# AllenNeuralDynamics/aind-smartspim-destripe

Hardware: AMD Instinct MI355X
Metric: 2048x2048 uint16 slices/s destriped (higher is better)
Workload: dtype f32

## Files before the change

### aind_smartspim_destripe_amd/csrc/dsx.hip

```cpp
#include <hip/hip_runtime.h>
#include <dlfcn.h>
#include <math.h>
#include <rccl/rccl.h>
#include <stdio.h>
#include <stdlib.h>
#include <string.h>

#include <string>
#include <vector>

#include "../../include/dsx.h"
#include "dsx_kernels.h"
#include "dsx_retile.h"
#include "dsx_rot90.h"
#include "dsx_pyramid.h"
#include "dsx_stackrank.h"
#include "dsx_volhist.h"
#include "dsx_project.h"
#include "dsx_wavelet.h"
#include "dsx_plan.h"
#include "dsx_chain.h"
#include "dsx_io.h"
#include "dsx_streaks.h"
#include "dsx_lightsheet.h"
// ... 402 lines not shown
  hipLaunchKernelGGL(dsx::k_hist, dim3(blocks, c.nb), dim3(64 * dsx::kHistWaves), 0, hs, a);
  DSX_HIP(hipGetLastError());
  return DSX_OK;
}

template <typename A>
void fill_fwd(A& a, const Chain& c, int l) {
  const dsx_ctx* ctx = c.ctx;
  const dsx::Plan& p = ctx->plan;
  const dsx::LevelPlan& lp = p.lv[l];
  memset(&a, 0, sizeof(a));
  a.in = c.d_in;
  a.in_plane_stride = (long long)p.H * p.W;
  a.ws = c.v.ws;
  a.ws_plane_stride = p.plane_floats;
  a.in_off = (l > 0) ? p.lv[l - 1].aa_off : 0;
  a.H = lp.hin; a.W = lp.win; a.ldin = lp.ldin;
  a.aa_off = lp.aa_off; a.da_off = lp.da_off;
  a.h = lp.h; a.w = lp.w; a.ld = lp.ld; a.lda = lp.lda;
  a.minmax = c.v.minmax;
  a.lvl = l; a.L = p.L;
  a.stats = c.v.stats;
  a.fg_cutoff = ctx->fg_cutoff;
  a.shared = ctx->stack_mode ? 1 : 0;
}

int stage_forward(const Chain& c) {
  dsx_ctx* ctx = c.ctx;
  const dsx::Plan& p = ctx->plan;
  const CohortView& v = c.v;
  const dsx::ChainShape& sh = c.sh;
  hipStream_t s = v.stream;
  const int nb = c.nb;
  for (int l = 0; l < p.L; ++l) {
    if (sh.fuse12 && l == 1) continue;
    if (l >= skips(ctx->tune).from) continue;
    const dsx::LevelPlan& lp = p.lv[l];
    LaunchScope ls(ctx, l == 0 ? KC_FWD1 : KC_FWD);
    if (sh.generic) {
      dsx::GenFwdArgs g;
      fill_fwd(g, c, l);
      g.F = ctx->wl_len;
      memcpy(g.lo, ctx->wl[0], sizeof(float) * ctx->wl_len);
      memcpy(g.hi, ctx->wl[1], sizeof(float) * ctx->wl_len);
      const dim3 gg((lp.w + dsx::kGenTW - 1) / dsx::kGenTW, (lp.h + dsx::kGenTH - 1) / dsx::kGenTH, nb);
      auto kern = level_kernel(l == 0, c.in_dtype, dsx::k_fwd_gen<2>, dsx::k_fwd_gen<0>, dsx::k_fwd_gen<1>);
      hipLaunchKernelGGL(kern, gg, dim3(256), dsx::gen_fwd_lds_bytes(g.F), s, g);
      DSX_HIP(hipGetLastError());
      continue;
    }
    dsx::Fwd1Args f;
    fill_fwd(f, c, l);
    f.ablate = ctx->ablate;
    f.fg_cutoff_u16 = (unsigned)std::min(65536.0, std::max(0.0, ceil((double)ctx->fg_cutoff)));
    const bool fused = sh.fuse12 && l == 0;
    if (fused) {
      const dsx::LevelPlan& l2 = p.lv[1];
      f.aa2_off = l2.aa_off; f.da2_off = l2.da_off;
      f.h2 = l2.h; f.w2 = l2.w; f.ld2 = l2.ld; f.lda2 = l2.lda;
    }
    const dsx::MarchLaunch m = dsx::fwd_launch(p, sh, ctx->tune, ctx->cus, nb, v.alone, l);
    f.nstrips = m.nstrips; f.nseg = m.nseg; f.rows_per_seg = m.rows_per_seg;
    auto kern = (fused && m.wpb == 8) ? pixel_kernel(c.in_dtype, dsx::k_fwd_march<0, true, 8>, dsx::k_fwd_march<1, true, 8>)
                : fused ? pixel_kernel(c.in_dtype, dsx::k_fwd_march<0, true>, dsx::k_fwd_march<1, true>)
                : level_kernel(l == 0, c.in_dtype, dsx::k_fwd_march<2>, dsx::k_fwd_march<0>, dsx::k_fwd_march<1>);
    hipLaunchKernelGGL(kern, dim3(m.grid_x, nb), dim3(64 * m.wpb), 0, s, f);
    DSX_HIP(hipGetLastError());
    if (sh.split && l == 0) {
      DSX_HIP(hipEventRecord(v.ev[0], s));
      DSX_HIP(hipStreamWaitEvent(v.helper, v.ev[0], 0));
      if (int rc = hist_levels(c, 0, 2, v.helper)) return rc;
      DSX_HIP(hipEventRecord(v.ev[1], v.helper));
    }
  }
  return DSX_OK;
}

int stage_thresholds(const Chain& c, int32_t* d_cfg_used) {
  dsx_ctx* ctx = c.ctx;
  const dsx::Plan& p = ctx->plan;
  const CohortView& v = c.v;
  hipStream_t s = v.stream;
  const int L = p.L;
  if (int rc = hist_levels(c, c.sh.split ? 2 : 0, L, s)) return rc;
  if (c.sh.split) DSX_HIP(hipStreamWaitEvent(s, v.ev[1], 0));
  if (L > 0 && c.sh.thresholds) {
    dsx::OtsuArgs a;
    a.stats = v.stats;
    a.npix = (double)p.H * (double)p.W;
    a.high_int = ctx->high_int;
    a.minmax = v.minmax;
    a.hist = v.hist;
    a.thr = v.thr;
    a.otsu = v.otsu;
    a.cfg = v.cfg;
    a.means = v.means;
    a.max_thr[0] = (float)ctx->cfg[0].max_threshold;
    a.max_thr[1] = (float)ctx->cfg[1].max_threshold;
    a.L = L;
    a.sticky = ctx->d_sticky;
    a.shared = ctx->stack_mode ? 1 : 0;
    LaunchScope ls(ctx, KC_OTSU);
    hipLaunchKernelGGL(dsx::k_otsu, dim3(L, c.nb), dim3(64), 0, s, a);
    DSX_HIP(hipGetLastError());
    if (d_cfg_used)
      DSX_HIP(hipMemcpyAsync(d_cfg_used, v.cfg, sizeof(int32_t) * c.nb, hipMemcpyDeviceToDevice, s));
  } else if (d_cfg_used) {
// ... 2477 lines not shown
```

### aind_smartspim_destripe_amd/csrc/dsx_chain.h

```cpp
#ifndef DSX_CHAIN_H
#define DSX_CHAIN_H

#include <stddef.h>
#include <stdlib.h>

#include <algorithm>

#include "dsx_plan.h"

namespace dsx {

constexpr int kMarchCols = 256;
constexpr int kMarchOut = (kMarchCols - 4) / 2;
constexpr int kFuseOut = (kMarchOut - 4) / 2;
constexpr int kHistWaves = 8;
constexpr int kRowMaxWaves = 8;
constexpr int kRowMultiMax = 8;
constexpr int kRowPackMax = 4;
constexpr int kRowPackValues = 18;
constexpr int kWideThreads = 512;
constexpr int kWideCpl = 36;
constexpr int kWideMaxLen = kWideThreads * kWideCpl;
constexpr int kRfWaves = 8;
constexpr int kRfRows = 2 * kRfWaves - 2;
constexpr int kGenTH = 16, kGenTW = 32;
constexpr int kGenOH = 32, kGenOW = 64;
constexpr size_t kLdsLimit = 160 * 1024;
constexpr size_t kC32Bytes = 8;

#ifdef __HIPCC__
#define DSX_CHAIN_HD __host__ __device__
#else
#define DSX_CHAIN_HD
#endif
inline DSX_CHAIN_HD int gen_fwd_cols(int F) { return 2 * kGenTW + F - 2 + 1; }
inline DSX_CHAIN_HD int gen_fwd_rows(int F) { return 2 * kGenTH + F - 2; }
inline size_t gen_fwd_lds_bytes(int F) {
  return sizeof(float) * (size_t)(gen_fwd_rows(F) + 2 * kGenTH) * gen_fwd_cols(F);
}
inline DSX_CHAIN_HD int gen_inv_krows(int F) { return kGenOH / 2 + F / 2 - 1; }
inline DSX_CHAIN_HD int gen_inv_kcols(int F) { return kGenOW / 2 + F / 2 - 1; }
inline size_t gen_inv_lds_bytes(int F) {
  return sizeof(float) * 2 * (size_t)gen_inv_krows(F) * (gen_inv_kcols(F) + 1 + kGenOW + 1);
}

}

struct DsxTuning {
  int row_wpb = 0;
  int march_waves = 256 * 16;
  bool no_quant = false;
  int seg_min_rows = 4;
  bool no_fuse = false;
  bool no_fuse_inv = false;
  bool no_pair = false;
  bool no_fuse_rf = false;
  bool fuse_rf_wide = false;
  int hist_rows = 0;
  int fwd_wpb = 8, inv_wpb = 8;
  bool no_row_multi = false;
  int row_multi_alone = 48;
  bool no_row_pack = false;
  int row_pack = 0;
  int row_pack_wpb = 4;
  int row_pack_fill = 16;
  int helper = -1;
  bool no_pipeline = false;
#ifdef DSX_DIAG
  int skip_hist = 0, skip_row = 0, skip_from = 1000;
#endif
};

namespace dsx {

inline int env_int(const char* name, int fallback) {
  const char* v = getenv(name);
  return (v && *v) ? atoi(v) : fallback;
}

inline void read_tuning(DsxTuning& t) {
  t.row_wpb = env_int("DSX_ROW_WPB", 0);
  if (t.row_wpb != 0) t.row_wpb = std::max(4, std::min(t.row_wpb, (int)kRowMaxWaves));
  t.march_waves = std::max(64, env_int("DSX_MARCH_WAVES", 256 * 16));
  t.no_quant = env_int("DSX_NO_QUANT", 0) != 0;
  t.seg_min_rows = std::max(2, env_int("DSX_SEG_MIN_ROWS", 4));
  t.no_fuse = env_int("DSX_NO_FUSE", 0) != 0;
  t.no_fuse_inv = env_int("DSX_NO_FUSE_INV", 0) != 0;
  t.no_pair = env_int("DSX_NO_PAIR", 0) != 0;
  t.no_fuse_rf = env_int("DSX_NO_FUSE_RF", 0) != 0;
  t.fuse_rf_wide = env_int("DSX_FUSE_RF_WIDE", 0) != 0;
  t.hist_rows = std::max(0, env_int("DSX_HIST_ROWS", 0));
  t.fwd_wpb = env_int("DSX_FWD_WPB", 8) == 4 ? 4 : 8;
  t.inv_wpb = env_int("DSX_INV_WPB", 8) == 4 ? 4 : 8;
  t.no_row_multi = env_int("DSX_NO_ROW_MULTI", 0) != 0;
  t.row_multi_alone = std::max(0, env_int("DSX_ROW_MULTI_ALONE", 48));
  t.no_row_pack = env_int("DSX_NO_ROW_PACK", 0) != 0;
  t.row_pack = std::max(0, std::min(env_int("DSX_ROW_PACK", 0), (int)kRowPackMax));
  t.row_pack_wpb = env_int("DSX_ROW_PACK_WPB", 4) == 8 ? 8 : 4;
  t.row_pack_fill = std::max(0, env_int("DSX_ROW_PACK_FILL", 16));
  t.helper = getenv("DSX_HELPER") ? (env_int("DSX_HELPER", 0) != 0 ? 1 : 0) : -1;
  t.no_pipeline = env_int("DSX_NO_PIPELINE", 0) != 0;
#ifdef DSX_DIAG
  t.skip_hist = env_int("DSX_SKIP_HIST", 0);
  t.skip_row = env_int("DSX_SKIP_ROW", 0);
  t.skip_from = env_int("DSX_SKIP_COARSE", 1000);
#endif
}

struct RowClass {
  bool wide;
  int cpl;
  int gf, nt, halo;
  int plan;
};

struct RowPlan {
  int M, radix[3];
  int cpl;
  int gf, nt, halo;
  bool swz;
};
constexpr int kRowPlanCount = 6;
constexpr RowPlan kRowPlans[kRowPlanCount] = {
    {1026, {19, 9, 6}, 18, 4, 1, 0, false},
    {1071, {17, 9, 7}, 18, 2, 1, 1, false},
    {2048, {16, 16, 8}, 36, 3, 4, 1, true},
    {1815, {15, 11, 11}, 36, 3, 3, 1, false},
    {1024, {16, 8, 8}, 18, 1, 4, 1, true},
    {960, {15, 8, 8}, 18, 1, 4, 1, false},
};
constexpr const RowPlan& row_plan(int id) { return kRowPlans[id - 1]; }

inline RowClass classify_row(int M, int w, int K, int npass, const int* radix) {
  RowClass c = {false, 0, -1, -1, -1, 0};
  const int cpl = (M + 63) / 64;
  if (cpl > 36) { c.wide = true; return c; }
  c.cpl = cpl_class(M);
  const int gf = w >> 8, nt = (w - (gf << 8) + 63) >> 6, halo = K > 0 ? 1 : 0;
  auto set = [&](int plan) { c.gf = gf; c.nt = nt; c.halo = halo; c.plan = plan; };
  for (int id = 1; id <= kRowPlanCount; ++id) {
    const RowPlan& p = row_plan(id);
    if (M == p.M && npass == 3 && radix[0] == p.radix[0] && radix[1] == p.radix[1] && radix[2] == p.radix[2] &&
        c.cpl == p.cpl && gf == p.gf && nt == p.nt && halo == p.halo) {
      set(id);
      return c;
    }
  }
  if (c.cpl == 18 && ((gf == 4 && nt == 1 && halo == 0) || (gf == 2 && nt == 1 && halo == 1))) set(0);
  return c;
}
inline RowClass classify_row(const LevelPlan& lp) { return classify_row(lp.M, lp.w, lp.K, lp.npass, lp.radix); }

inline int rowfinal_plan(const Plan& p, bool in_u16, bool out_u16, bool pair_io, bool wide) {
  const LevelPlan& lp = p.lv[0];
// ... 253 lines not shown
```

### aind_smartspim_destripe_amd/csrc/dsx_kernels.h

```cpp
#ifndef DSX_KERNELS_H
#define DSX_KERNELS_H

#include <type_traits>
#include <hip/hip_runtime.h>
#include <stdint.h>

#include "dsx_chain.h"
#include "dsx_fft_core.h"

#ifdef DSX_DIAG
#define DSX_ABL(a, bits) (((a).ablate & (bits)) != 0)
#else
#define DSX_ABL(a, bits) false
#endif

namespace dsx {

constexpr int kMaxLevels = 16;
constexpr int kMaxPasses = 16;
constexpr int kWave = 64;

#define DSX_DEC_LO                                                                              \
  {0.03522629188570953f, -0.08544127388202666f, -0.13501102001025458f, 0.45987750211849154f,   \
   0.8068915093110925f,  0.33267055295008263f}
// ... 105 lines not shown
}
__device__ __forceinline__ unsigned bit_select(int m, unsigned a, unsigned b) {
  unsigned r;
  asm("v_bfi_b32 %0, %1, %2, %3" : "=v"(r) : "v"(m), "v"(a), "v"(b));
  return r;
}
__device__ __forceinline__ int odd_lane_mask(int lane) {
  int m = -(lane & 1);
  asm("" : "+v"(m));
  return m;
}
__device__ __forceinline__ float bit_select(int m, float a, float b) {
  return as_f32(bit_select(m, as_u32(a), as_u32(b)));
}

__device__ __forceinline__ void wave_sync() {
  __builtin_amdgcn_fence(__ATOMIC_RELEASE, "wavefront");
  __builtin_amdgcn_wave_barrier();
  __builtin_amdgcn_fence(__ATOMIC_ACQUIRE, "wavefront");
}

__device__ __forceinline__ float lane_above(float v) {
  return __builtin_bit_cast(float, __builtin_amdgcn_update_dpp(0, __builtin_bit_cast(int, v), 0x130, 0xF, 0xF, true));
}

__global__ __launch_bounds__(256) void k_zero3(uint4* p0, int n0, uint4* p1, int n1, uint4* p2, int n2) {
  const uint4 z = make_uint4(0u, 0u, 0u, 0u);
  for (int i = blockIdx.x * 256 + threadIdx.x; i < n0 + n1 + n2; i += gridDim.x * 256) {
    if (i < n0) p0[i] = z;
    else if (i < n0 + n1) p1[i - n0] = z;
    else p2[i - n0 - n1] = z;
  }
}

struct Fwd1Args {
  const void* in;
  long long in_plane_stride;
  float* ws;
  long long ws_plane_stride;
  long long in_off;
  int H, W, ldin;
  long long aa_off, da_off;
  int h, w, ld, lda;
  unsigned* minmax;
  int lvl, L;
  PlaneStats* stats;
  float fg_cutoff;
  unsigned fg_cutoff_u16;
  int nstrips, nseg, rows_per_seg;
  long long aa2_off, da2_off;
  int h2, w2, ld2, lda2;
  int ablate;
  int shared;
};

constexpr int kRingRows = 8;
constexpr int kRingPitch = 128;

template <int IN_KIND>
struct MarchStats {
  unsigned cnt = 0;
  unsigned isum_all = 0, isum_fg = 0;
  double fsum_all = 0.0, fsum_fg = 0.0;
  unsigned bad = 0;
  __device__ __forceinline__ void add(float f, float cutoff) {
    if (IN_KIND != 0) bad |= (f > -1.0f && f <= 3.402823466e38f) ? 0u : 1u;
    if (IN_KIND == 0) {
      const unsigned u = (unsigned)f;
      isum_all += u;
      if (f >= cutoff) { isum_fg += u; cnt++; }
    } else {
      fsum_all += (double)f;
      if (f >= cutoff) { fsum_fg += (double)f; cnt++; }
    }
  }
};

struct MarchRaw {
  float4 f;
};

struct MarchCol {
  int gc0;
  int base;
  bool vec;
  bool rev;
  bool dead;
  bool own;
  unsigned own_mask[2];
  int rc[4];
};

__device__ __forceinline__ MarchCol march_col(int gc0, int W, int ld, int w_out, bool lane_owns, bool ext) {
  MarchCol c;
  c.gc0 = gc0;
  c.own = lane_owns;
  c.dead = gc0 > 2 * w_out - 1;
  c.rev = false;
  c.base = gc0;
  const bool aligned = (ld & 3) == 0;
  c.vec = aligned && gc0 >= 0 && gc0 + 3 < W;
  if (ext && aligned && gc0 >= -4 && gc0 + 3 < W + 8) c.vec = true;
  if (!c.vec && !ext && aligned && (W & 3) == 0) {
    if (gc0 + 3 < 0 && -gc0 - 1 < W) { c.base = -gc0 - 4; c.rev = true; c.vec = true; }
    else if (gc0 >= W && 2 * W - 4 - gc0 >= 0) { c.base = 2 * W - 4 - gc0; c.rev = true; c.vec = true; }
  }
// ... 23 lines not shown
      r.f = make_float4(__uint_as_float(u.x), __uint_as_float(u.y), 0.f, 0.f);
    } else {
      const dsx_u32x4 u = __builtin_amdgcn_raw_buffer_load_b128(rs, voff, soff, 0);
      r.f = make_float4(__uint_as_float(u.x), __uint_as_float(u.y), __uint_as_float(u.z), __uint_as_float(u.w));
    }
    return r;
  }
};

template <int IN_KIND, bool FAST>
__device__ __forceinline__ MarchRaw march_issue(const MarchSrc<IN_KIND>& ms, int ld, int H, int gr_raw,
                                                const MarchCol& c) {
  MarchRaw r;
  if (FAST)
    return ms.load((unsigned)(reflect_idx(gr_raw, H) * ld) * MarchSrc<IN_KIND>::ES);
  const void* src = ms.src;
  const long long row = (long long)reflect_idx(gr_raw, H) * ld;
  r.f = make_float4(0.f, 0.f, 0.f, 0.f);
  if (c.dead) return r;
  if (IN_KIND == 0) {
    const uint16_t* p = (const uint16_t*)src + row;
    if (c.vec) {
      const uint2 u = *(const uint2*)(p + c.base);
      r.f.x = __uint_as_float(u.x);
      r.f.y = __uint_as_float(u.y);
    } else {
      const unsigned u0 = p[c.rc[0]], u1 = p[c.rc[1]], u2 = p[c.rc[2]], u3 = p[c.rc[3]];
      r.f.x = __uint_as_float(u0 | (u1 << 16));
      r.f.y = __uint_as_float(u2 | (u3 << 16));
    }
  } else {
    const float* p = (const float*)src + row;
    if (c.vec) r.f = *(const float4*)(p + c.base);
    else r.f = make_float4(p[c.rc[0]], p[c.rc[1]], p[c.rc[2]], p[c.rc[3]]);
  }
  return r;
}

template <int IN_KIND>
__device__ __forceinline__ void march_issue6(const MarchSrc<IN_KIND>& ms, int ld, int H, int g0, const MarchCol& c,
                                             MarchRaw (&out)[6]) {
  constexpr int ES = MarchSrc<IN_KIND>::ES;
  if (g0 >= 0 && g0 + 5 < H) {
    const unsigned pitch = (unsigned)ld * ES;
    unsigned soff = (unsigned)g0 * pitch;
#pragma unroll
    for (int r = 0; r < 6; ++r, soff += pitch) out[r] = ms.load(soff);
  } else {
#pragma unroll
    for (int r = 0; r < 6; ++r) out[r] = march_issue<IN_KIND, true>(ms, ld, H, g0 + r, c);
  }
}

template <int IN_KIND, bool INSIDE = false>
__device__ __forceinline__ void march_consume(const Fwd1Args& a, const MarchRaw& r, int gr_raw, const MarchCol& c,
                                              bool row_in_seg, bool any_rev, MarchStats<IN_KIND>& st,
                                              float (&x)[4]) {
  if (IN_KIND == 0) {
    unsigned u0 = __float_as_uint(r.f.x), u1 = __float_as_uint(r.f.y);
    if (any_rev) {
      if (c.rev) {
        const unsigned t = u0;
        u0 = (u1 >> 16) | (u1 << 16);
        u1 = (t >> 16) | (t << 16);
      }
    }
    if (row_in_seg && (INSIDE || (gr_raw >= 0 && gr_raw < a.H))) {
      const unsigned o0 = u0 & c.own_mask[0], o1 = u1 & c.own_mask[1];
      st.isum_all = __builtin_amdgcn_sad_u16(o1, 0u, __builtin_amdgcn_sad_u16(o0, 0u, st.isum_all));
      typedef unsigned short dsx_u16x2 __attribute__((ext_vector_type(2)));
      union { unsigned u; dsx_u16x2 v; } pa, pb, pm;
      pa.u = o0; pb.u = o1;
      pm.v = __builtin_elementwise_max(pa.v, pb.v);
      const unsigned m = max(pm.u & 0xFFFFu, pm.u >> 16);
      if (m >= a.fg_cutoff_u16) {
        const unsigned px[4] = {o0 & 0xFFFFu, o0 >> 16, o1 & 0xFFFFu, o1 >> 16};
#pragma unroll
        for (int e = 0; e < 4; ++e)
          if (px[e] >= a.fg_cutoff_u16) { st.isum_fg += px[e]; st.cnt++; }
      }
    }
    const dsx_f2 one = {1.0f, 1.0f};
    const dsx_f2 p01 = dsx_f2{(float)(u0 & 0xFFFFu), (float)(u0 >> 16)} + one;
    const dsx_f2 p23 = dsx_f2{(float)(u1 & 0xFFFFu), (float)(u1 >> 16)} + one;
    x[0] = __builtin_amdgcn_logf(p01.x);
    x[1] = __builtin_amdgcn_logf(p01.y);
    x[2] = __builtin_amdgcn_logf(p23.x);
    x[3] = __builtin_amdgcn_logf(p23.y);
    return;
  }
  float v[4] = {r.f.x, r.f.y, r.f.z, r.f.w};
  if (any_rev && c.vec && c.rev) {
    const float t0 = v[0], t1 = v[1];
    v[0] = v[3]; v[1] = v[2]; v[2] = t1; v[3] = t0;
  }
  if (IN_KIND == 2) {
    x[0] = v[0]; x[1] = v[1]; x[2] = v[2]; x[3] = v[3];
    return;
  }
  const bool own_row = row_in_seg && c.own && (INSIDE || (gr_raw >= 0 && gr_raw < a.H));
#pragma unroll
  for (int e = 0; e < 4; ++e) {
    if (own_row && c.gc0 + e >= 0 && c.gc0 + e < a.W) st.add(v[e], a.fg_cutoff);
    x[e] = __builtin_amdgcn_logf(1.0f + v[e]);
  }
}

struct FuseGeom {
  int o2;
  int j0;
  int own2_lo;
  int own1_lo, own1_hi;
};
// ... 10 lines not shown
template <int IN_KIND, bool FAST, bool FUSE, bool EDGE = true>
__device__ __forceinline__ void fwd_march_body(const Fwd1Args& a, float (*s_ring)[kRingRows][kRingPitch], int lane, int wave,
                                               int strip, int seg, int plane, const MarchCol& col, bool any_rev_in) {
  const bool any_rev = EDGE && any_rev_in;
  constexpr float LO[6] = DSX_DEC_LO;
  constexpr float HI[6] = DSX_DEC_HI;
  constexpr float KS = (IN_KIND == 2) ? 1.0f : 0.69314718055994530942f;
  constexpr float LOV[6] = {LO[0] * KS, LO[1] * KS, LO[2] * KS, LO[3] * KS, LO[4] * KS, LO[5] * KS};
  constexpr float HIV[6] = {HI[0] * KS, HI[1] * KS, HI[2] * KS, HI[3] * KS, HI[4] * KS, HI[5] * KS};
  const FuseGeom fg = FUSE ? fuse_geom(a, strip) : FuseGeom();
  const int i2b = seg * a.rows_per_seg;
  const int i2e = FUSE ? min(a.h2, i2b + a.rows_per_seg) : 0;
  const int i_first = (FUSE && i2e == a.h2) ? min(2 * i2b - 4, (a.h - 6) & ~1) : 2 * i2b - 4;
  const int i_begin = FUSE ? max(0, i_first) : seg * a.rows_per_seg;
  const int i_end = FUSE ? min(a.h, 2 * i2e) : min(a.h, i_begin + a.rows_per_seg);
  const int own_row_lo = FUSE ? 2 * i2b : i_begin;
  const int steady_lo = max(own_row_lo, 6);
  const int steady_hi = min(min(i_end, a.h - 2), (a.H - 2) >> 1);
  const int j0 = FUSE ? fg.j0 : kMarchOut * strip;
  int next2 = i2b;
  float q2min = __builtin_huge_valf(), q2max = 0.f;
  float* aa2 = FUSE ? a.ws + plane * a.ws_plane_stride + a.aa2_off : nullptr;
  float* da2 = FUSE ? a.ws + plane * a.ws_plane_stride + a.da2_off : nullptr;
  const void* src;
  if (IN_KIND == 0) src = (const uint16_t*)a.in + plane * a.in_plane_stride;
  else if (IN_KIND == 1) src = (const float*)a.in + plane * a.in_plane_stride;
  else src = a.ws + plane * a.ws_plane_stride + a.in_off;
  const MarchSrc<IN_KIND> ms(src, col);
  constexpr bool PAIRLD = FUSE && FAST && !EDGE && IN_KIND == 0;
  const bool odd_lane = (lane & 1) != 0;
  const int oddm = odd_lane_mask(lane);
  const unsigned pitch_b = (unsigned)a.ldin * 2u;
  const unsigned voff_pair0 = (unsigned)(col.base - (odd_lane ? 4 : 0)) * 2u;
  const unsigned voff_pair = voff_pair0 + (odd_lane ? pitch_b : 0u);
  auto issue_pairs = [&](int g0, MarchRaw (&out)[6]) {
    if (g0 >= 0 && g0 + 5 < a.H) {
      unsigned soff = (unsigned)g0 * pitch_b;
#pragma unroll
      for (int p = 0; p < 3; ++p, soff += 2u * pitch_b) {
        const dsx_u32x4 u = __builtin_amdgcn_raw_buffer_load_b128(ms.rs, voff_pair, soff, 0);
        out[2 * p].f = make_float4(__uint_as_float(u.x), __uint_as_float(u.y), __uint_as_float(u.z), __uint_as_float(u.w));
      }
    } else {
#pragma unroll
      for (int p = 0; p < 3; ++p) {
        const int re = reflect_idx(g0 + 2 * p, a.H), ro = reflect_idx(g0 + 2 * p + 1, a.H);
        const dsx_u32x4 u = __builtin_amdgcn_raw_buffer_load_b128(ms.rs, voff_pair0 + (unsigned)(odd_lane ? ro : re) * pitch_b, 0u, 0);
        out[2 * p].f = make_float4(__uint_as_float(u.x), __uint_as_float(u.y), __uint_as_float(u.z), __uint_as_float(u.w));
      }
    }
  };
  float* aa = a.ws + plane * a.ws_plane_stride + a.aa_off;
  float* da = a.ws + plane * a.ws_plane_stride + a.da_off;
  const __amdgpu_buffer_rsrc_t rs_da = dsx_rsrc(da), rs_aa2 = dsx_rsrc(aa2), rs_da2 = dsx_rsrc(da2);

  MarchStats<IN_KIND> st;
  float win[6][4];
  {
    MarchRaw pr[4];
#pragma unroll
    for (int r = 0; r < 4; ++r) pr[r] = march_issue<IN_KIND, FAST>(ms, a.ldin, a.H, 2 * i_begin - 4 + r, col);
#pragma unroll
    for (int r = 0; r < 4; ++r) march_consume<IN_KIND>(a, pr[r], 2 * i_begin - 4 + r, col, false, any_rev, st, win[r]);
  }

  float qmin = __builtin_huge_valf(), qmax = 0.f;
  const int jj0 = 2 * lane;
  const bool out_lane = lane < kMarchOut / 2;
  const bool edge_strip = EDGE && ((j0 <= 0) || (j0 + kMarchOut >= a.w - 8));

  const int jl = j0 + jj0;
  const bool c_v0 = FUSE && (!EDGE || (jl >= 0 && jl < a.w)), c_v1 = FUSE && (!EDGE || (jl + 1 >= 0 && jl + 1 < a.w));
  const bool c_s0 = FUSE && out_lane && jl >= fg.own1_lo && jl < fg.own1_hi;
  const bool c_s1 = EDGE ? (FUSE && out_lane && jl + 1 >= fg.own1_lo && jl + 1 < fg.own1_hi) : c_s0;
  const unsigned off_da = (unsigned)max(jl, 0) * 4u + ((FUSE && DSX_ABL(a, 64)) ? 24u * (unsigned)strip : 0u);
  const int jo2 = fg.o2 + lane;
  const bool l2_valid = FUSE && lane < kFuseOut && (!EDGE || jo2 < a.w2);
  const bool l2_store = l2_valid && jo2 >= fg.own2_lo;
  const bool l2_edge = FUSE && EDGE && (fg.o2 == 0 || fg.o2 + kFuseOut >= a.w2 - 8);
  const unsigned off_2 = (unsigned)jo2 * 4u;

  auto l2_step = [&](auto steady_c, int i2) {
    constexpr bool STEADY = decltype(steady_c)::value;
    dsx_f2 c[6];
    if (EDGE) wave_sync();
#pragma unroll
    for (int k = 0; k < 6; ++k) {
      int r = 2 * i2 - 4 + k;
      if (!STEADY) r = r < 0 ? -1 - r : (r >= a.h ? 2 * a.h - 1 - r : r);
      c[k] = *(const dsx_f2*)&s_ring[wave][r & (kRingRows - 1)][jj0];
    }
    dsx_f2 lo2 = LO[0] * c[5], hi2 = HI[0] * c[5];
#pragma unroll
    for (int k = 1; k < 6; ++k) {
      lo2 = pk_fma(LO[k], c[5 - k], lo2);
      hi2 = pk_fma(HI[k], c[5 - k], hi2);
    }
    dsx_f4 pk = {lo2.x, hi2.x, lo2.y, hi2.y};
    const dsx_f4 p0 = pk;
    const dsx_f4 p1 = {lane_above(p0.x), lane_above(p0.y), lane_above(p0.z), lane_above(p0.w)};
    const dsx_f4 p2 = {lane_above(p1.x), lane_above(p1.y), lane_above(p1.z), lane_above(p1.w)};
    dsx_f2 v = LO[5] * p0.xy;
    v = pk_fma(LO[4], p0.zw, v);
    v = pk_fma(LO[3], p1.xy, v);
    v = pk_fma(LO[2], p1.zw, v);
    v = pk_fma(LO[1], p2.xy, v);
    v = pk_fma(LO[0], p2.zw, v);
    const float q = v.y * v.y;
    q2min = min_no_nan(q2min, l2_valid ? q : __builtin_huge_valf());
    q2max = max_no_nan(q2max, l2_valid ? q : 0.f);
    if (l2_store && !DSX_ABL(a, 16 | 128)) {
      __builtin_amdgcn_raw_buffer_store_b32(__float_as_uint(v.x), rs_aa2, off_2, (unsigned)(i2 * a.lda2) * 4u, 0);
      __builtin_amdgcn_raw_buffer_store_b32(__float_as_uint(v.y), rs_da2, off_2, (unsigned)(i2 * a.ld2) * 4u, 0);
      if (l2_edge) {
        float* arow = aa2 + (long long)i2 * a.lda2;
        if (jo2 < 4) arow[-1 - jo2] = v.x;
        if (jo2 >= a.w2 - 8) arow[2 * a.w2 - 1 - jo2] = v.x;
      }
    }
  };

  auto step = [&](auto steady_c, int i, const MarchRaw& raw0, const MarchRaw& raw1, float (&r0)[4], float (&r1)[4],
                  float (&r2)[4], float (&r3)[4], float (&r4)[4], float (&r5)[4]) {
    constexpr bool STEADY = decltype(steady_c)::value;
    const bool own_row = STEADY || !FUSE || i >= own_row_lo;
    march_consume<IN_KIND, STEADY>(a, raw0, 2 * i, col, own_row, any_rev, st, r4);
    march_consume<IN_KIND, STEADY>(a, raw1, 2 * i + 1, col, own_row, any_rev, st, r5);
    float lo[4], hi[4];
#pragma unroll
    for (int e = 0; e < 4; ++e) {
      lo[e] = LOV[0] * r5[e];
      hi[e] = HIV[0] * r5[e];
      lo[e] = fmaf(LOV[1], r4[e], lo[e]); hi[e] = fmaf(HIV[1], r4[e], hi[e]);
      lo[e] = fmaf(LOV[2], r3[e], lo[e]); hi[e] = fmaf(HIV[2], r3[e], hi[e]);
      lo[e] = fmaf(LOV[3], r2[e], lo[e]); hi[e] = fmaf(HIV[3], r2[e], hi[e]);
      lo[e] = fmaf(LOV[4], r1[e], lo[e]); hi[e] = fmaf(HIV[4], r1[e], hi[e]);
      lo[e] = fmaf(LOV[5], r0[e], lo[e]); hi[e] = fmaf(HIV[5], r0[e], hi[e]);
    }
    float res[2][2];
    {
      float v0l, v1l, v0h, v1h;
      const float c0 = LO[0], c1 = LO[1], c2 = LO[2], c3 = LO[3];
#define DSX_DPP_UP " wave_shl:1 row_mask:0xf bank_mask:0xf bound_ctrl:1\n"
      asm("s_nop 1\n"
          "v_mul_f32_dpp %0, %5, %12" DSX_DPP_UP
          "v_mul_f32_dpp %1, %7, %12" DSX_DPP_UP
          "v_mul_f32_dpp %2, %9, %12" DSX_DPP_UP
          "v_mul_f32_dpp %3, %11, %12" DSX_DPP_UP
          "v_fmac_f32_dpp %0, %4, %13" DSX_DPP_UP
          "v_fmac_f32_dpp %1, %6, %13" DSX_DPP_UP
          "v_fmac_f32_dpp %2, %8, %13" DSX_DPP_UP
          "v_fmac_f32_dpp %3, %10, %13" DSX_DPP_UP
          "v_fmac_f32_dpp %1, %5, %14" DSX_DPP_UP
          "v_fmac_f32_dpp %3, %9, %14" DSX_DPP_UP
          "v_fmac_f32_dpp %1, %4, %15" DSX_DPP_UP
          "v_fmac_f32_dpp %3, %8, %15" DSX_DPP_UP
          : "=&v"(v0l), "=&v"(v1l), "=&v"(v0h), "=&v"(v1h)
          : "v"(lo[0]), "v"(lo[1]), "v"(lo[2]), "v"(lo[3]), "v"(hi[0]), "v"(hi[1]), "v"(hi[2]), "v"(hi[3]),
            "v"(c0), "v"(c1), "v"(c2), "v"(c3));
#undef DSX_DPP_UP
      v0l = fmaf(LO[2], lo[3], v0l); v0l = fmaf(LO[3], lo[2], v0l); v0l = fmaf(LO[4], lo[1], v0l); v0l = fmaf(LO[5], lo[0], v0l);
      v1l = fmaf(LO[4], lo[3], v1l); v1l = fmaf(LO[5], lo[2], v1l);
      v0h = fmaf(LO[2], hi[3], v0h); v0h = fmaf(LO[3], hi[2], v0h); v0h = fmaf(LO[4], hi[1], v0h); v0h = fmaf(LO[5], hi[0], v0h);
      v1h = fmaf(LO[4], hi[3], v1h); v1h = fmaf(LO[5], hi[2], v1h);
      res[0][0] = v0l; res[0][1] = v1l; res[1][0] = v0h; res[1][1] = v1h;
    }
    if (FUSE) {
      if (out_lane) {
        const int j = jl;
        const float q0 = res[1][0] * res[1][0], q1 = res[1][1] * res[1][1];
        if (own_row && !DSX_ABL(a, 16 | 256)) {
          const unsigned soff = DSX_ABL(a, 64) ? (unsigned)i * 4224u : (unsigned)(i * a.ld) * 4u;
          if (c_s0 && c_s1) {
            const dsx_u32x2 dv = {__float_as_uint(res[1][0]), __float_as_uint(res[1][1])};
            __builtin_amdgcn_raw_buffer_store_b64(dv, rs_da, off_da, soff, kBufNT);
          } else {
            if (c_s0) __builtin_amdgcn_raw_buffer_store_b32(__float_as_uint(res[1][0]), rs_da, off_da, soff, kBufNT);
            if (c_s1) __builtin_amdgcn_raw_buffer_store_b32(__float_as_uint(res[1][1]), rs_da, off_da + 4u, soff, kBufNT);
          }
        }
        qmin = min_no_nan(qmin, min_no_nan(c_v0 ? q0 : __builtin_huge_valf(), c_v1 ? q1 : __builtin_huge_valf()));
        qmax = max_no_nan(qmax, max_no_nan(c_v0 ? q0 : 0.f, c_v1 ? q1 : 0.f));
        float* ring = s_ring[wave][i & (kRingRows - 1)];
        if (!edge_strip) {
          *(float2*)(ring + jj0) = make_float2(res[0][0], res[0][1]);
        } else {
#pragma unroll
          for (int e = 0; e < 2; ++e) {
            const int je = j + e;
            if (je >= 0 && je < a.w) {
              ring[jj0 + e] = res[0][e];
              if (je < 4 && -1 - je - j0 >= 0) ring[-1 - je - j0] = res[0][e];
              const int t = 2 * a.w - 1 - je - j0;
              if (je >= a.w - 6 && t < kRingPitch) ring[t] = res[0][e];
            }
          }
        }
      }
      if (STEADY) {
        if (2 * next2 + 1 <= i) {
          l2_step(std::true_type(), next2);
          ++next2;
        }
      } else {
        while (next2 < i2e) {
          const int need = min(max(2 * next2 + 1, 3 - 2 * next2), a.h - 1);
          if (need > i) break;
          l2_step(std::false_type(), next2);
          ++next2;
        }
      }
    } else
    if (out_lane) {
      const int j = j0 + jj0;
      const long long o = (long long)i * a.ld + j;
      const long long oa = (long long)i * a.lda + j;
      float* arow = aa + (long long)i * a.lda;
      if (j + 1 < a.w) {
        *(float2*)(aa + oa) = make_float2(res[0][0], res[0][1]);
        *(float2*)(da + o) = make_float2(res[1][0], res[1][1]);
        const float q0 = res[1][0] * res[1][0], q1 = res[1][1] * res[1][1];
        qmin = min_no_nan(qmin, min_no_nan(q0, q1));
        qmax = max_no_nan(qmax, max_no_nan(q0, q1));
      } else if (j < a.w) {
        aa[oa] = res[0][0];
        da[o] = res[1][0];
        const float q0 = res[1][0] * res[1][0];
        qmin = min_no_nan(qmin, q0);
        qmax = max_no_nan(qmax, q0);
      }
      if (edge_strip) {
#pragma unroll
        for (int e = 0; e < 2; ++e) {
          const int je = j + e;
          if (je < a.w) {
            if (je < 4) arow[-1 - je] = res[0][e];
            if (je >= a.w - 8) arow[2 * a.w - 1 - je] = res[0][e];
          }
        }
      }
    }
  };

  constexpr int DEPTH = (IN_KIND == 0) ? 2 : 1;
  MarchRaw nxt[DEPTH][6];
#pragma unroll
  for (int d = 0; d < DEPTH; ++d) {
    if (PAIRLD) {
      issue_pairs(2 * (i_begin + 3 * d), nxt[d]);
    } else if (FAST) {
      march_issue6<IN_KIND>(ms, a.ldin, a.H, 2 * (i_begin + 3 * d), col, nxt[d]);
    } else {
#pragma unroll
      for (int r = 0; r < 6; ++r)
        nxt[d][r] = march_issue<IN_KIND, FAST>(ms, a.ldin, a.H, 2 * (i_begin + 3 * d) + r, col);
    }
  }
  auto group = [&](auto steady_c, int i) {
    constexpr bool STEADY = decltype(steady_c)::value;
    MarchRaw cur[6];
#pragma unroll
    for (int r = 0; r < 6; ++r) cur[r] = nxt[0][r];
    if (PAIRLD) {
#pragma unroll
      for (int p = 0; p < 3; ++p) {
        const unsigned x = __float_as_uint(nxt[0][2 * p].f.x), y = __float_as_uint(nxt[0][2 * p].f.y);
        const unsigned z = __float_as_uint(nxt[0][2 * p].f.z), w = __float_as_uint(nxt[0][2 * p].f.w);
        const unsigned gx = swap_adjacent(bit_select(oddm, x, z)), gy = swap_adjacent(bit_select(oddm, y, w));
        cur[2 * p].f.x = __uint_as_float(bit_select(oddm, gx, x));
        cur[2 * p].f.y = __uint_as_float(bit_select(oddm, gy, y));
        cur[2 * p + 1].f.x = __uint_as_float(bit_select(oddm, z, gx));
        cur[2 * p + 1].f.y = __uint_as_float(bit_select(oddm, w, gy));
      }
    }
#pragma unroll
    for (int d = 0; d + 1 < DEPTH; ++d)
#pragma unroll
      for (int r = 0; r < 6; ++r) nxt[d][r] = nxt[d + 1][r];
    if (i + 3 * DEPTH < i_end) {
      if (PAIRLD) {
        issue_pairs(2 * (i + 3 * DEPTH), nxt[DEPTH - 1]);
      } else if (FAST) {
        march_issue6<IN_KIND>(ms, a.ldin, a.H, 2 * (i + 3 * DEPTH), col, nxt[DEPTH - 1]);
      } else {
#pragma unroll
        for (int r = 0; r < 6; ++r)
          nxt[DEPTH - 1][r] = march_issue<IN_KIND, FAST>(ms, a.ldin, a.H, 2 * (i + 3 * DEPTH) + r, col);
      }
    }
    if (STEADY) {
      step(std::true_type(), i, cur[0], cur[1], win[0], win[1], win[2], win[3], win[4], win[5]);
      step(std::true_type(), i + 1, cur[2], cur[3], win[2], win[3], win[4], win[5], win[0], win[1]);
      step(std::true_type(), i + 2, cur[4], cur[5], win[4], win[5], win[0], win[1], win[2], win[3]);
    } else {
      step(std::false_type(), i, cur[0], cur[1], win[0], win[1], win[2], win[3], win[4], win[5]);
      if (i + 1 < i_end) step(std::false_type(), i + 1, cur[2], cur[3], win[2], win[3], win[4], win[5], win[0], win[1]);
      if (i + 2 < i_end) step(std::false_type(), i + 2, cur[4], cur[5], win[4], win[5], win[0], win[1], win[2], win[3]);
    }
  };
  const bool steady_on = FUSE && !EDGE;
  {
    int i = i_begin;
    int run_lo = i_end, run_hi = i_end;
    if (steady_on) {
      run_lo = i_begin + 3 * ((max(steady_lo - i_begin, 0) + 2) / 3);
      run_hi = (steady_hi - run_lo >= 3) ? run_lo + 3 * ((steady_hi - run_lo) / 3) : run_lo;
      if (run_hi == run_lo) run_lo = run_hi = i_end;
    }
#pragma nounroll
    for (int part = 0; part < 2; ++part) {
      const int stop = part == 0 ? min(run_lo, i_end) : i_end;
      for (; i < stop; i += 3) group(std::false_type(), i);
      if (part == 0)
        for (; i < run_hi; i += 3) group(std::true_type(), i);
    }
  }

  qmin = wave_min_f32(qmin);
  qmax = wave_max_f32(qmax);
  if (lane == 0 && qmin <= qmax) {
    unsigned* mm = a.minmax + ((long long)(a.shared ? 0 : plane) * a.L + a.lvl) * 2;
    atomicMax(&mm[0], ~as_u32(qmin));
    atomicMax(&mm[1], as_u32(qmax));
  }
  if (FUSE) {
    q2min = wave_min_f32(q2min);
    q2max = wave_max_f32(q2max);
    if (lane == 0 && q2min <= q2max) {
      unsigned* mm = a.minmax + ((long long)(a.shared ? 0 : plane) * a.L + a.lvl + 1) * 2;
      atomicMax(&mm[0], ~as_u32(q2min));
      atomicMax(&mm[1], as_u32(q2max));
    }
  }
  if (IN_KIND != 2) {
    double s_all, s_fg;
    if (IN_KIND == 0) {
      s_all = (double)st.isum_all;
      s_fg = (double)st.isum_fg;
    } else {
      s_all = st.fsum_all;
      s_fg = st.fsum_fg;
    }
    s_all = wave_sum_f64(s_all);
    s_fg = wave_sum_f64(s_fg);
    const unsigned cnt = __reduce_add_sync(~0ull, st.cnt);
    const bool bad_any = (IN_KIND == 1) && __any(st.bad != 0u) != 0;
    if (lane == 0) {
      PlaneStats* ps = a.stats + plane;
      if (s_all != 0.0) atomicAdd(&ps->sum_all, s_all);
      if (cnt != 0) {
        atomicAdd(&ps->sum_fg, s_fg);
        atomicAdd(&ps->cnt_fg, (unsigned long long)cnt);
      }
      if (IN_KIND == 1 && bad_any) atomicOr(&ps->flags, 1ull);
    }
  }
}

constexpr int kFwdMinWaves = 4;
template <int IN_KIND, bool FUSE = false, int WPB = 4>
__global__ __launch_bounds__(64 * WPB, (FUSE && IN_KIND == 0) ? kFwdMinWaves : 1) void k_fwd_march(Fwd1Args a) {
  __shared__ __attribute__((aligned(16))) float s_ring[FUSE ? WPB : 1][kRingRows][FUSE ? kRingPitch : 4];
  const int lane = threadIdx.x & 63;
  const int wave = __builtin_amdgcn_readfirstlane(threadIdx.x >> 6);
  const int item = blockIdx.x * WPB + wave;
  if (item >= a.nstrips * a.nseg) return;
  const int strip = item % a.nstrips, seg = item / a.nstrips;
  const int plane = blockIdx.y;
  if (seg * a.rows_per_seg >= (FUSE ? a.h2 : a.h)) return;
  if (FUSE) {
    const FuseGeom fg = fuse_geom(a, strip);
    const int gc0 = 2 * fg.j0 - 4 + 4 * lane;
    const bool owns = gc0 >= 4 * kFuseOut * strip && (strip == a.nstrips - 1 || gc0 < 4 * kFuseOut * (strip + 1));
    MarchCol col = march_col(gc0, a.W, a.ldin, a.w, owns, false);
    if (!col.vec) { col.dead = true; col.base = 0; col.rev = false; }
    const bool any_rev = __any(col.rev) != 0;
    const bool interior = strip > 0 && strip < a.nstrips - 1 && fg.j0 > 0 && fg.j0 + kMarchOut + 2 < a.w - 8 &&
                          fg.o2 + kFuseOut < a.w2 - 8 && __all(col.vec && !col.rev && !col.dead) != 0;
    float (*ring)[kRingRows][kRingPitch] = (float (*)[kRingRows][kRingPitch])s_ring;
    if (interior) fwd_march_body<IN_KIND, true, true, false>(a, ring, lane, wave, strip, seg, plane, col, false);
    else fwd_march_body<IN_KIND, true, true, true>(a, ring, lane, wave, strip, seg, plane, col, any_rev);
    return;
  }
  const MarchCol col = march_col(2 * kMarchOut * strip - 4 + 4 * lane, a.W, a.ldin, a.w, lane >= 1, IN_KIND == 2);
  const bool all_vec = __all(col.vec || (col.dead && a.W >= 4 && (a.ldin & 3) == 0)) != 0;
  const bool any_rev = __any(col.rev) != 0;
  if (all_vec) fwd_march_body<IN_KIND, true, false>(a, nullptr, lane, wave, strip, seg, plane, col, any_rev);
  else fwd_march_body<IN_KIND, false, false>(a, nullptr, lane, wave, strip, seg, plane, col, any_rev);
}

struct HistArgs {
  const float* ws;
  long long ws_plane_stride;
  const unsigned* minmax;
  unsigned* hist;
  int L;
  int shared;
  int nlev;
  int lvl[kMaxLevels];
  long long da_off[kMaxLevels];
  int h[kMaxLevels], w[kMaxLevels], ld[kMaxLevels];
  int rows_per_block[kMaxLevels];
  int blk_end[kMaxLevels];
};

struct HistBins {
  float qmin, qmax, scale;
  double first64, step64;
  __device__ __forceinline__ HistBins(float lo, float hi) : qmin(lo), qmax(hi) {
    scale = 256.0f / (qmax - qmin);
    first64 = (double)qmin;
    step64 = ((double)qmax - (double)qmin) / 256.0;
  }
  __device__ __forceinline__ float edge(int i) const { return (float)__dadd_rn(__dmul_rn((double)i, step64), first64); }
};

constexpr int kHistLoads = 8;

__global__ __launch_bounds__(64 * kHistWaves) void k_hist(HistArgs args) {
  __shared__ __attribute__((aligned(16))) unsigned s_cnt[256 * 32];
  __shared__ float s_edge[264];
  const int tid = threadIdx.x, lane = tid & 63;
// ... 2040 lines not shown
```

Before: 74450.

## Add steady-state fast path for edge strips in fused forward march kernel

Edge strips of the fused level-1/level-2 forward wavelet march now get a steady-state loop. It uses bounded buffer resources so out-of-range stores are dropped by hardware, select-based reversal of the u16 word order, and mirror-reflected input loads in place of per-row branching. The level-2 step is scheduled at compile time by row parity over 6-row groups. The aim is to remove the branchy general edge path, which may dominate the tail of the launch for boundary strips. It adds code size and register pressure, relies on buffer bounds checking for correctness, and can be disabled through an environment flag.

```diff
diff --git a/aind_smartspim_destripe_amd/csrc/dsx.hip b/aind_smartspim_destripe_amd/csrc/dsx.hip
--- a/aind_smartspim_destripe_amd/csrc/dsx.hip
+++ b/aind_smartspim_destripe_amd/csrc/dsx.hip
@@ -478,7 +478,8 @@
     dsx::Fwd1Args f;
     fill_fwd(f, c, l);
     f.ablate = ctx->ablate;
-    f.fg_cutoff_u16 = (unsigned)std::min(65536.0, std::max(0.0, ceil((double)ctx->fg_cutoff)));
+    f.edge_general = ctx->tune.fwd_edge_general ? 1 : 0;
+    f.fg_cutoff_u16 =(unsigned)std::min(65536.0, std::max(0.0, ceil((double)ctx->fg_cutoff)));
     const bool fused = sh.fuse12 && l == 0;
     if (fused) {
       const dsx::LevelPlan& l2 = p.lv[1];
diff --git a/aind_smartspim_destripe_amd/csrc/dsx_chain.h b/aind_smartspim_destripe_amd/csrc/dsx_chain.h
--- a/aind_smartspim_destripe_amd/csrc/dsx_chain.h
+++ b/aind_smartspim_destripe_amd/csrc/dsx_chain.h
@@ -66,6 +66,7 @@
   int row_pack_fill = 16;
   int helper = -1;
   bool no_pipeline = false;
+  bool fwd_edge_general = false;
 #ifdef DSX_DIAG
   int skip_hist = 0, skip_row = 0, skip_from = 1000;
 #endif
@@ -100,6 +101,7 @@
   t.row_pack_fill = std::max(0, env_int("DSX_ROW_PACK_FILL", 16));
   t.helper = getenv("DSX_HELPER") ? (env_int("DSX_HELPER", 0) != 0 ? 1 : 0) : -1;
   t.no_pipeline = env_int("DSX_NO_PIPELINE", 0) != 0;
+  t.fwd_edge_general = env_int("DSX_FWD_EDGE_GENERAL", 0) != 0;
 #ifdef DSX_DIAG
   t.skip_hist = env_int("DSX_SKIP_HIST", 0);
   t.skip_row = env_int("DSX_SKIP_ROW", 0);
diff --git a/aind_smartspim_destripe_amd/csrc/dsx_kernels.h b/aind_smartspim_destripe_amd/csrc/dsx_kernels.h
--- a/aind_smartspim_destripe_amd/csrc/dsx_kernels.h
+++ b/aind_smartspim_destripe_amd/csrc/dsx_kernels.h
@@ -181,6 +181,7 @@
   int h2, w2, ld2, lda2;
   int ablate;
   int shared;
+  int edge_general;
 };
 
 constexpr int kRingRows = 8;
@@ -310,13 +311,17 @@
   }
 }
 
-template <int IN_KIND, bool INSIDE = false>
+template <int IN_KIND, bool INSIDE = false, bool SELREV = false>
 __device__ __forceinline__ void march_consume(const Fwd1Args& a, const MarchRaw& r, int gr_raw, const MarchCol& c,
                                               bool row_in_seg, bool any_rev, MarchStats<IN_KIND>& st,
                                               float (&x)[4]) {
   if (IN_KIND == 0) {
     unsigned u0 = __float_as_uint(r.f.x), u1 = __float_as_uint(r.f.y);
-    if (any_rev) {
+    if (SELREV) {
+      const unsigned s0 = (u1 >> 16) | (u1 << 16), s1 = (u0 >> 16) | (u0 << 16);
+      u0 = c.rev ? s0 : u0;
+      u1 = c.rev ? s1 : u1;
+    } else if (any_rev) {
       if (c.rev) {
         const unsigned t = u0;
         u0 = (u1 >> 16) | (u1 << 16);
@@ -433,7 +438,13 @@
   };
   float* aa = a.ws + plane * a.ws_plane_stride + a.aa_off;
   float* da = a.ws + plane * a.ws_plane_stride + a.da_off;
-  const __amdgpu_buffer_rsrc_t rs_da = dsx_rsrc(da), rs_aa2 = dsx_rsrc(aa2), rs_da2 = dsx_rsrc(da2);
+  const long long da_bytes = (long long)a.h * a.ld * 4, aa2_bytes = ((long long)a.h2 * a.lda2 + 8) * 4, da2_bytes = (long long)a.h2 * a.ld2 * 4;
+  const bool bounded = FUSE && EDGE && max(da_bytes, max(aa2_bytes, da2_bytes)) <= (long long)kBufDiscard;
+  constexpr unsigned kAa2Bias = (FUSE && EDGE) ? 16u : 0u;
+  const __amdgpu_buffer_rsrc_t rs_da = __builtin_amdgcn_make_buffer_rsrc((void*)da, 0, bounded ? (int)da_bytes : -1, 0x00020000);
+  const __amdgpu_buffer_rsrc_t rs_aa2 =
+      __builtin_amdgcn_make_buffer_rsrc((void*)((const char*)aa2 - kAa2Bias), 0, bounded ? (int)aa2_bytes : -1, 0x00020000);
+  const __amdgpu_buffer_rsrc_t rs_da2 = __builtin_amdgcn_make_buffer_rsrc((void*)da2, 0, bounded ? (int)da2_bytes : -1, 0x00020000);
 
   MarchStats<IN_KIND> st;
   float win[6][4];
@@ -460,9 +471,25 @@
   const bool l2_store = l2_valid && jo2 >= fg.own2_lo;
   const bool l2_edge = FUSE && EDGE && (fg.o2 == 0 || fg.o2 + kFuseOut >= a.w2 - 8);
   const unsigned off_2 = (unsigned)jo2 * 4u;
-
-  auto l2_step = [&](auto steady_c, int i2) {
+  const unsigned off_2a = off_2 + kAa2Bias;
+
+  const bool es_da = out_lane && c_s0 && c_s1;
+  const bool es_ml = l2_store && l2_edge && jo2 < 4, es_mr = l2_store && l2_edge && jo2 >= a.w2 - 8;
+  const unsigned es_off_da = (es_da && !DSX_ABL(a, 16 | 256)) ? off_da : kBufDiscard;
+  const unsigned es_off_aa2 = (l2_store && !DSX_ABL(a, 16 | 128)) ? off_2a : kBufDiscard;
+  const unsigned es_off_da2 = (l2_store && !DSX_ABL(a, 16 | 128)) ? off_2 : kBufDiscard;
+  const unsigned es_off_m = DSX_ABL(a, 16 | 128) ? kBufDiscard
+                            : es_ml ? (unsigned)(3 - jo2) * 4u
+                            : es_mr ? (unsigned)(2 * a.w2 - 1 - jo2 + 4) * 4u : kBufDiscard;
+  const bool es_v0 = out_lane && c_v0, es_v1 = out_lane && c_v1;
+  const bool es_left = fg.o2 == 0;
+  const bool es_right = strip == a.nstrips - 1 || fg.j0 + kMarchOut + 2 >= a.w - 8 || fg.o2 + kFuseOut >= a.w2 - 8;
+  const bool es_ok = FUSE && EDGE && IN_KIND == 0 && bounded && a.edge_general == 0 && es_left != es_right && !DSX_ABL(a, 64) &&
+                     __all((c_s0 == c_s1) && !(es_ml && es_mr)) != 0;
+
+  auto l2_step = [&](auto steady_c, auto es_c, int i2) {
     constexpr bool STEADY = decltype(steady_c)::value;
+    constexpr bool ES = decltype(es_c)::value;
     dsx_f2 c[6];
     if (EDGE) wave_sync();
 #pragma unroll
@@ -490,8 +517,14 @@
     const float q = v.y * v.y;
     q2min = min_no_nan(q2min, l2_valid ? q : __builtin_huge_valf());
     q2max = max_no_nan(q2max, l2_valid ? q : 0.f);
+    if (ES) {
+      const unsigned soff_a = (unsigned)(i2 * a.lda2) * 4u;
+      __builtin_amdgcn_raw_buffer_store_b32(__float_as_uint(v.x), rs_aa2, es_off_aa2, soff_a, 0);
+      __builtin_amdgcn_raw_buffer_store_b32(__float_as_uint(v.y), rs_da2, es_off_da2, (unsigned)(i2 * a.ld2) * 4u, 0);
+      __builtin_amdgcn_raw_buffer_store_b32(__float_as_uint(v.x), rs_aa2, es_off_m, soff_a, 0);
+    } else
     if (l2_store && !DSX_ABL(a, 16 | 128)) {
-      __builtin_amdgcn_raw_buffer_store_b32(__float_as_uint(v.x), rs_aa2, off_2, (unsigned)(i2 * a.lda2) * 4u, 0);
+      __builtin_amdgcn_raw_buffer_store_b32(__float_as_uint(v.x), rs_aa2, off_2a, (unsigned)(i2 * a.lda2) * 4u, 0);
       __builtin_amdgcn_raw_buffer_store_b32(__float_as_uint(v.y), rs_da2, off_2, (unsigned)(i2 * a.ld2) * 4u, 0);
       if (l2_edge) {
         float* arow = aa2 + (long long)i2 * a.lda2;
@@ -501,12 +534,14 @@
     }
   };
 
-  auto step = [&](auto steady_c, int i, const MarchRaw& raw0, const MarchRaw& raw1, float (&r0)[4], float (&r1)[4],
+  auto step = [&](auto steady_c, auto l2_c, int i, const MarchRaw& raw0, const MarchRaw& raw1, float (&r0)[4], float (&r1)[4],
                   float (&r2)[4], float (&r3)[4], float (&r4)[4], float (&r5)[4]) {
     constexpr bool STEADY = decltype(steady_c)::value;
+    constexpr int L2K = decltype(l2_c)::value;
+    constexpr bool ES = L2K >= 0;
     const bool own_row = STEADY || !FUSE || i >= own_row_lo;
-    march_consume<IN_KIND, STEADY>(a, raw0, 2 * i, col, own_row, any_rev, st, r4);
-    march_consume<IN_KIND, STEADY>(a, raw1, 2 * i + 1, col, own_row, any_rev, st, r5);
+    march_consume<IN_KIND, STEADY, ES>(a, raw0, 2 * i, col, own_row, any_rev, st, r4);
+    march_consume<IN_KIND, STEADY, ES>(a, raw1, 2 * i + 1, col, own_row, any_rev, st, r5);
     float lo[4], hi[4];
 #pragma unroll
     for (int e = 0; e < 4; ++e) {
@@ -546,6 +581,28 @@
       v1h = fmaf(LO[4], hi[3], v1h); v1h = fmaf(LO[5], hi[2], v1h);
       res[0][0] = v0l; res[0][1] = v1l; res[1][0] = v0h; res[1][1] = v1h;
     }
+    if (FUSE && ES) {
+      const float q0 = res[1][0] * res[1][0], q1 = res[1][1] * res[1][1];
+      const dsx_u32x2 dv = {__float_as_uint(res[1][0]), __float_as_uint(res[1][1])};
+      __builtin_amdgcn_raw_buffer_store_b64(dv, rs_da, es_off_da, (unsigned)(i * a.ld) * 4u, kBufNT);
+      qmin = min_no_nan(qmin, min_no_nan(es_v0 ? q0 : __builtin_huge_valf(), es_v1 ? q1 : __builtin_huge_valf()));
+      qmax = max_no_nan(qmax, max_no_nan(es_v0 ? q0 : 0.f, es_v1 ? q1 : 0.f));
+      float* ring = s_ring[wave][i & (kRingRows - 1)];
+#pragma unroll
+      for (int e = 0; e < 2; ++e) {
+        const int je = jl + e;
+        const int tl = -1 - je - j0, tr = 2 * a.w - 1 - je - j0;
+        if (out_lane && je >= 0 && je < a.w) {
+          ring[jj0 + e] = res[0][e];
+          if (je < 4 && tl >= 0) ring[tl] = res[0][e];
+          if (je >= a.w - 6 && tr < kRingPitch) ring[tr] = res[0][e];
+        }
+      }
+      if (L2K == 1) {
+        l2_step(std::true_type(), std::true_type(), next2);
+        ++next2;
+      }
+    } else
     if (FUSE) {
       if (out_lane) {
         const int j = jl;
@@ -580,14 +637,14 @@
       }
       if (STEADY) {
         if (2 * next2 + 1 <= i) {
-          l2_step(std::true_type(), next2);
+          l2_step(std::true_type(), std::false_type(), next2);
           ++next2;
         }
       } else {
         while (next2 < i2e) {
           const int need = min(max(2 * next2 + 1, 3 - 2 * next2), a.h - 1);
           if (need > i) break;
-          l2_step(std::false_type(), next2);
+          l2_step(std::false_type(), std::false_type(), next2);
           ++next2;
         }
       }
@@ -637,8 +694,10 @@
         nxt[d][r] = march_issue<IN_KIND, FAST>(ms, a.ldin, a.H, 2 * (i_begin + 3 * d) + r, col);
     }
   }
-  auto group = [&](auto steady_c, int i) {
+  auto group = [&](auto steady_c, auto par_c, int i) {
     constexpr bool STEADY = decltype(steady_c)::value;
+    constexpr int PAR = decltype(par_c)::value;
+    constexpr bool ES = PAR >= 0;
     MarchRaw cur[6];
 #pragma unroll
     for (int r = 0; r < 6; ++r) cur[r] = nxt[0][r];
@@ -658,6 +717,12 @@
     for (int d = 0; d + 1 < DEPTH; ++d)
 #pragma unroll
       for (int r = 0; r < 6; ++r) nxt[d][r] = nxt[d + 1][r];
+    if (ES) {
+      const int g0 = 2 * (i + 3 * DEPTH);
+#pragma unroll
+      for (int r = 0; r < 6; ++r)
+        nxt[DEPTH - 1][r] = ms.load((unsigned)min(g0 + r, 2 * a.H - 1 - g0 - r) * pitch_b);
+    } else
     if (i + 3 * DEPTH < i_end) {
       if (PAIRLD) {
         issue_pairs(2 * (i + 3 * DEPTH), nxt[DEPTH - 1]);
@@ -669,31 +734,48 @@
           nxt[DEPTH - 1][r] = march_issue<IN_KIND, FAST>(ms, a.ldin, a.H, 2 * (i + 3 * DEPTH) + r, col);
       }
     }
-    if (STEADY) {
-      step(std::true_type(), i, cur[0], cur[1], win[0], win[1], win[2], win[3], win[4], win[5]);
-      step(std::true_type(), i + 1, cur[2], cur[3], win[2], win[3], win[4], win[5], win[0], win[1]);
-      step(std::true_type(), i + 2, cur[4], cur[5], win[4], win[5], win[0], win[1], win[2], win[3]);
+    constexpr std::integral_constant<int, -1> dyn;
+    if (ES) {
+      step(std::true_type(), std::integral_constant<int, PAR == 1 ? 1 : 0>(), i, cur[0], cur[1], win[0], win[1], win[2], win[3], win[4], win[5]);
+      step(std::true_type(), std::integral_constant<int, PAR == 0 ? 1 : 0>(), i + 1, cur[2], cur[3], win[2], win[3], win[4], win[5], win[0], win[1]);
+      step(std::true_type(), std::integral_constant<int, PAR == 1 ? 1 : 0>(), i + 2, cur[4], cur[5], win[4], win[5], win[0], win[1], win[2], win[3]);
+    } else if (STEADY) {
+      step(std::true_type(), dyn, i, cur[0], cur[1], win[0], win[1], win[2], win[3], win[4], win[5]);
+      step(std::true_type(), dyn, i + 1, cur[2], cur[3], win[2], win[3], win[4], win[5], win[0], win[1]);
+      step(std::true_type(), dyn, i + 2, cur[4], cur[5], win[4], win[5], win[0], win[1], win[2], win[3]);
     } else {
-      step(std::false_type(), i, cur[0], cur[1], win[0], win[1], win[2], win[3], win[4], win[5]);
-      if (i + 1 < i_end) step(std::false_type(), i + 1, cur[2], cur[3], win[2], win[3], win[4], win[5], win[0], win[1]);
-      if (i + 2 < i_end) step(std::false_type(), i + 2, cur[4], cur[5], win[4], win[5], win[0], win[1], win[2], win[3]);
+      step(std::false_type(), dyn, i, cur[0], cur[1], win[0], win[1], win[2], win[3], win[4], win[5]);
+      if (i + 1 < i_end) step(std::false_type(), dyn, i + 1, cur[2], cur[3], win[2], win[3], win[4], win[5], win[0], win[1]);
+      if (i + 2 < i_end) step(std::false_type(), dyn, i + 2, cur[4], cur[5], win[4], win[5], win[0], win[1], win[2], win[3]);
     }
   };
-  const bool steady_on = FUSE && !EDGE;
+  const bool steady_on = FUSE && (!EDGE || es_ok);
   {
     int i = i_begin;
     int run_lo = i_end, run_hi = i_end;
     if (steady_on) {
       run_lo = i_begin + 3 * ((max(steady_lo - i_begin, 0) + 2) / 3);
       run_hi = (steady_hi - run_lo >= 3) ? run_lo + 3 * ((steady_hi - run_lo) / 3) : run_lo;
+      if (EDGE) {
+        run_lo += 3 * (run_lo & 1);
+        run_hi = run_lo + 6 * (max(run_hi - run_lo, 0) / 6);
+      }
       if (run_hi == run_lo) run_lo = run_hi = i_end;
     }
 #pragma nounroll
     for (int part = 0; part < 2; ++part) {
       const int stop = part == 0 ? min(run_lo, i_end) : i_end;
-      for (; i < stop; i += 3) group(std::false_type(), i);
-      if (part == 0)
-        for (; i < run_hi; i += 3) group(std::true_type(), i);
+      for (; i < stop; i += 3) group(std::false_type(), std::integral_constant<int, -1>(), i);
+      if (part == 0) {
+        if (EDGE) {
+          for (; i < run_hi; i += 6) {
+            group(std::true_type(), std::integral_constant<int, (FUSE && EDGE) ? 0 : -1>(), i);
+            group(std::true_type(), std::integral_constant<int, (FUSE && EDGE) ? 1 : -1>(), i + 3);
+          }
+        } else {
+          for (; i < run_hi; i += 3) group(std::true_type(), std::integral_constant<int, -1>(), i);
+        }
+      }
     }
   }
 
@@ -746,9 +828,11 @@
   const int wave = __builtin_amdgcn_readfirstlane(threadIdx.x >> 6);
   const int item = blockIdx.x * WPB + wave;
   if (item >= a.nstrips * a.nseg) return;
-  const int strip = item % a.nstrips, seg = item / a.nstrips;
+  int strip = item % a.nstrips;
+  const int seg = item / a.nstrips;
   const int plane = blockIdx.y;
   if (seg * a.rows_per_seg >= (FUSE ? a.h2 : a.h)) return;
+  if (FUSE && DSX_ABL(a, 512) && a.nstrips >= 3) strip = min(max(strip, 1), a.nstrips - 2);
   if (FUSE) {
     const FuseGeom fg = fuse_geom(a, strip);
     const int gc0 = 2 * fg.j0 - 4 + 4 * lane;
```

After: 75340, median of 6. +1.2%, better.
